# yassouali/pytorch-segmentation

Measured on NVIDIA H100. Metric: images/sec DeepLabV3+/ResNet101 513x513 train step (fwd+CE+bwd+SGD), higher is better.
Workload: dtype bf16

## Files before the change

### pytorch-segmentation_b200/csrc/seg_loss.cu

```cuda
#include "seg_common.cuh"

namespace seg {

__device__ __forceinline__ void block_accum2(double a, double b, double* out) {
  a = warp_sum_d(a);
  b = warp_sum_d(b);
  __shared__ double sa[32], sb[32];
  const int lane = threadIdx.x & 31, warp = threadIdx.x >> 5;
  if (lane == 0) {
    sa[warp] = a;
    sb[warp] = b;
  }
  __syncthreads();
  if (warp == 0) {
    const int nw = (blockDim.x + 31) >> 5;
    a = lane < nw ? sa[lane] : 0.0;
    b = lane < nw ? sb[lane] : 0.0;
    a = warp_sum_d(a);
    b = warp_sum_d(b);
    if (lane == 0) {
      atomicAdd(out, a);
      atomicAdd(out + 1, b);
    }
  }
// ... 93 lines not shown
                                                            int N, int C, int H, int W, double* accum) {
  const int64_t HW = (int64_t)H * W, total = (int64_t)N * HW;
  double inter = 0.0, psum = 0.0;
  for (int64_t i = blockIdx.x * (int64_t)blockDim.x + threadIdx.x; i < total; i += (int64_t)gridDim.x * blockDim.x) {
    const int64_t t = target[i];
    const int n = (int)(i / HW);
    const float* l = logits + (int64_t)n * C * HW + (i - (int64_t)n * HW);
    float mx = -INFINITY;
    for (int c = 0; c < C; ++c) mx = fmaxf(mx, l[(int64_t)c * HW]);
    float se = 0.f, et = 0.f;
    for (int c = 0; c < C; ++c) {
      const float e = expf(l[(int64_t)c * HW] - mx);
      se += e;
      if (c == t) et = e;
    }
    inter += (double)(et / se);
    psum += 1.0;
  }
  block_accum2(inter, psum, accum);
}

__global__ void __launch_bounds__(256) dice_nchw_bwd_kernel(const float* __restrict__ logits, const int64_t* __restrict__ target,
                                                            int N, int C, int H, int W, const double* __restrict__ accum,
                                                            float smooth, const float* __restrict__ gscale,
                                                            float* __restrict__ dl, float beta) {
  const int64_t HW = (int64_t)H * W, total = (int64_t)N * HW;
  const double D = accum[1] + accum[1] + (double)smooth;
  const float g = (gscale ? *gscale : 1.f) * (float)(-2.0 / D);
  for (int64_t i = blockIdx.x * (int64_t)blockDim.x + threadIdx.x; i < total; i += (int64_t)gridDim.x * blockDim.x) {
    const int64_t t = target[i];
    const int n = (int)(i / HW);
    const int64_t off = (int64_t)n * C * HW + (i - (int64_t)n * HW);
    const float* l = logits + off;
    float* d = dl + off;
    float mx = -INFINITY;
    for (int c = 0; c < C; ++c) mx = fmaxf(mx, l[(int64_t)c * HW]);
    float se = 0.f;
    for (int c = 0; c < C; ++c) se += expf(l[(int64_t)c * HW] - mx);
    const float inv = 1.f / se;
    const float pt = (t >= 0 && t < C) ? expf(l[t * HW] - mx) * inv : 0.f;
    for (int c = 0; c < C; ++c) {
      const float pc = expf(l[(int64_t)c * HW] - mx) * inv;
      const float v = g * pt * ((c == t ? 1.f : 0.f) - pc);
      d[(int64_t)c * HW] = (beta != 0.f) ? beta * d[(int64_t)c * HW] + v : v;
    }
  }
}

__global__ void dice_finalize_kernel(const double* accum, float smooth, float* loss) {
  if (threadIdx.x == 0 && blockIdx.x == 0)
    *loss = (float)(1.0 - (2.0 * accum[0] + smooth) / (accum[1] + accum[1] + smooth));
}

__global__ void loss_finalize_kernel(const double* accum, int mean, float* loss) {
  if (threadIdx.x == 0 && blockIdx.x == 0) *loss = (float)(!mean ? accum[0] : accum[1] > 0.0 ? accum[0] / accum[1] : 0.0);
}

struct Lerp2 {
  int i0, i1;
  float l1;
};
__device__ __forceinline__ Lerp2 src_idx(int dst, float scale, int in_size, int ac) {
  float s;
  if (ac) {
    s = scale * (float)dst;
  } else {
    s = scale * ((float)dst + 0.5f) - 0.5f;
    if (s < 0.f) s = 0.f;
  }
  Lerp2 r;
  r.i0 = (int)s;
  if (r.i0 > in_size - 1) r.i0 = in_size - 1;
  r.i1 = r.i0 + ((r.i0 < in_size - 1) ? 1 : 0);
  r.l1 = s - (float)r.i0;
  return r;
}
static inline float rscale(int in_size, int out_size, int ac) {
  if (ac) return out_size > 1 ? (float)(in_size - 1) / (float)(out_size - 1) : 0.f;
  return (float)in_size / (float)out_size;
}

constexpr int MAXC = 160;
constexpr int TILE = 32;

__device__ __forceinline__ double ce_grad_scale(double gmax, float sh, float sw, int Ho, int Wo) {
  const double ry = sh > 0.f ? 2.0 / sh : (double)Ho, rx = sw > 0.f ? 2.0 / sw : (double)Wo;
  int e;
  frexp(fabs(gmax) * (ry + 2.0) * (rx + 2.0), &e);
  return ldexp(1.0, 61 - e);
}
__device__ __forceinline__ float warp_weight_max(const float* w, int C) {
  float m = w ? 0.f : 1.f;
  if (w)
    for (int c = threadIdx.x & 31; c < C; c += 32) m = fmaxf(m, w[c]);
  for (int o = 16; o > 0; o >>= 1) m = fmaxf(m, __shfl_xor_sync(0xffffffffu, m, o));
  return m;
}
template <int K>
__device__ __forceinline__ double loss_grad_bound(float g, const LossArgs& la, int C) {
  if (K == LOSS_CE) return (double)g;
  return (double)g * (double)warp_weight_max(la.weight, C) * (K == LOSS_FOCAL ? 1.0 + (double)la.gamma : 1.0);
}
__device__ __forceinline__ unsigned long long to_fixed(float v, double scale) {
  return (unsigned long long)__double2ll_rn((double)v * scale);
}

template <bool BWD, int K, bool MET = false>
__global__ void __launch_bounds__(256) upsample_ce_kernel(const float* __restrict__ lo, const int64_t* __restrict__ target,
                                                          int N, int Hi, int Wi, int Ho, int Wo, int C, int ac, float sh,
                                                          float sw, int64_t ignore, LossArgs la, double* accum, int32_t* argmax,
                                                          const float* __restrict__ gscale,
                                                          unsigned long long* __restrict__ dlo_fixed, int patch, int tile,
                                                          unsigned long long* __restrict__ counters) {
  extern __shared__ unsigned long long sm64[];
  unsigned long long* dst = BWD ? sm64 : nullptr;
  float* src = reinterpret_cast<float*>(BWD ? sm64 + patch * patch * C : sm64);
  unsigned int* hist = MET ? reinterpret_cast<unsigned int*>(src + patch * patch * C) : nullptr;
  const int tiles_x = (Wo + tile - 1) / tile, tiles_y = (Ho + tile - 1) / tile;
  int t = blockIdx.x;
  const int tx = t % tiles_x;
  t /= tiles_x;
  const int ty = t % tiles_y;
  const int n = t / tiles_y;
  const int oy0 = ty * tile, ox0 = tx * tile;
  const int oy1 = min(oy0 + tile, Ho) - 1, ox1 = min(ox0 + tile, Wo) - 1;
  const int sy0 = src_idx(oy0, sh, Hi, ac).i0, sx0 = src_idx(ox0, sw, Wi, ac).i0;
  const int sy1 = src_idx(oy1, sh, Hi, ac).i1, sx1 = src_idx(ox1, sw, Wi, ac).i1;
  const int ph = sy1 - sy0 + 1, pw = sx1 - sx0 + 1;
  for (int i = threadIdx.x; i < ph * pw * C; i += blockDim.x) {
    const int c = i % C;
    const int pp = i / C;
    const int py = pp / pw, px = pp - py * pw;
    src[i] = lo[(((int64_t)n * Hi + sy0 + py) * Wi + sx0 + px) * C + c];
    if (BWD) dst[i] = 0ull;
  }
  if (MET)
    for (int i = threadIdx.x; i < 3 * C + 2; i += blockDim.x) hist[i] = 0u;
  __syncthreads();
  double loss = 0.0, cnt = 0.0;
  unsigned int n_correct = 0u, n_labeled = 0u;
  float g = 0.f;
  double scale = 0.0;
  if (BWD) {
    g = loss_grad_g<K>(gscale, accum, la.mean);
    scale = ce_grad_scale(loss_grad_bound<K>(g, la, C), sh, sw, Ho, Wo);
  }
  for (int e = threadIdx.x; e < tile * tile; e += blockDim.x) {
    const int oy = oy0 + e / tile, ox = ox0 + e % tile;
    if (oy >= Ho || ox >= Wo) continue;
    const int64_t tg = target[((int64_t)n * Ho + oy) * Wo + ox];
    const bool valid = tg != ignore;
    const bool labeled = MET && tg >= 0 && tg < C;
    if (K == LOSS_FOCAL && !BWD) cnt += 1.0;
    if (!valid && (BWD || (argmax == nullptr && !labeled))) continue;
    const Lerp2 ly = src_idx(oy, sh, Hi, ac), lx = src_idx(ox, sw, Wi, ac);
    const float h1 = ly.l1, h0 = 1.f - h1, w1 = lx.l1, w0 = 1.f - w1;
    const float* pa = src + ((ly.i0 - sy0) * pw + (lx.i0 - sx0)) * C;
    const float* pb = src + ((ly.i0 - sy0) * pw + (lx.i1 - sx0)) * C;
    const float* pc = src + ((ly.i1 - sy0) * pw + (lx.i0 - sx0)) * C;
    const float* pd = src + ((ly.i1 - sy0) * pw + (lx.i1 - sx0)) * C;
    float mx = -INFINITY;
    int am = 0;
    for (int c = 0; c < C; ++c) {
      const float v = h0 * (w0 * pa[c] + w1 * pb[c]) + h1 * (w0 * pc[c] + w1 * pd[c]);
      if (v > mx) {
        mx = v;
        am = c;
      }
    }
    float se = 0.f, lt = 0.f;
    for (int c = 0; c < C; ++c) {
      const float v = h0 * (w0 * pa[c] + w1 * pb[c]) + h1 * (w0 * pc[c] + w1 * pd[c]);
      se += expf(v - mx);
      if (c == tg) lt = v;
    }
    if (!BWD) {
      if (argmax) argmax[((int64_t)n * Ho + oy) * Wo + ox] = am;
      if (MET && labeled) {
        ++n_labeled;
        atomicAdd(&hist[2 + C + am], 1u);
        atomicAdd(&hist[2 + 2 * C + (int)tg], 1u);
        if (am == (int)tg) {
          ++n_correct;
          atomicAdd(&hist[2 + (int)tg], 1u);
        }
      }
      if (valid) {
        const float w = K == LOSS_CE ? 1.f : class_weight(la, tg, C);
        loss += (double)pixel_loss<K>(mx + logf(se) - lt, w, la.gamma);
        if (K == LOSS_CE) cnt += 1.0;
        if (K == LOSS_WCE) cnt += (double)w;
      }
    } else {
      const float inv = 1.f / se;
      const float gp = K == LOSS_CE ? g : g * pixel_grad_factor<K>(mx + logf(se) - lt, class_weight(la, tg, C), la.gamma);
      unsigned long long* da = dst + ((ly.i0 - sy0) * pw + (lx.i0 - sx0)) * C;
      unsigned long long* db = dst + ((ly.i0 - sy0) * pw + (lx.i1 - sx0)) * C;
      unsigned long long* dc = dst + ((ly.i1 - sy0) * pw + (lx.i0 - sx0)) * C;
      unsigned long long* dd = dst + ((ly.i1 - sy0) * pw + (lx.i1 - sx0)) * C;
      for (int c = 0; c < C; ++c) {
        const float v = h0 * (w0 * pa[c] + w1 * pb[c]) + h1 * (w0 * pc[c] + w1 * pd[c]);
        const float gr = (expf(v - mx) * inv - (c == tg ? 1.f : 0.f)) * gp;
        atomicAdd(da + c, to_fixed(h0 * w0 * gr, scale));
        atomicAdd(db + c, to_fixed(h0 * w1 * gr, scale));
        atomicAdd(dc + c, to_fixed(h1 * w0 * gr, scale));
        atomicAdd(dd + c, to_fixed(h1 * w1 * gr, scale));
      }
    }
  }
  if (!BWD) {
    block_accum2(loss, cnt, accum);
    if (MET) {
      n_correct = __reduce_add_sync(0xffffffffu, n_correct);
      n_labeled = __reduce_add_sync(0xffffffffu, n_labeled);
      if ((threadIdx.x & 31) == 0) {
        atomicAdd(&hist[0], n_correct);
        atomicAdd(&hist[1], n_labeled);
      }
      __syncthreads();
      for (int i = threadIdx.x; i < 3 * C + 2; i += blockDim.x) {
        const unsigned int v = hist[i];
        if (v != 0u) atomicAdd(counters + i, (unsigned long long)v);
      }
    }
  } else {
    __syncthreads();
    for (int i = threadIdx.x; i < ph * pw * C; i += blockDim.x) {
      const unsigned long long v = dst[i];
      if (v != 0ull) {
        const int c = i % C;
        const int pp = i / C;
        const int py = pp / pw, px = pp - py * pw;
        atomicAdd(dlo_fixed + (((int64_t)n * Hi + sy0 + py) * Wi + sx0 + px) * C + c, v);
      }
    }
  }
}

template <int K>
__global__ void ce_grad_from_fixed_kernel(const unsigned long long* __restrict__ acc, int64_t n, const float* gscale,
                                          const double* accum, LossArgs la, int C, float sh, float sw, int Ho, int Wo,
                                          float* __restrict__ dlo) {
  const double inv = 1.0 / ce_grad_scale(loss_grad_bound<K>(loss_grad_g<K>(gscale, accum, la.mean), la, C), sh, sw, Ho, Wo);
  for (int64_t i = blockIdx.x * (int64_t)blockDim.x + threadIdx.x; i < n; i += (int64_t)gridDim.x * blockDim.x)
    dlo[i] = (float)((double)(long long)acc[i] * inv);
}

__device__ __forceinline__ float logit_f(__nv_bfloat16 v) { return bf2f(v); }
__device__ __forceinline__ float logit_f(float v) { return v; }
template <bool BWD, int K, bool MET = false, typename T = __nv_bfloat16>
__global__ void __launch_bounds__(256) shuffle_ce_kernel(const T* __restrict__ lo, int ldlo,
                                                         const int64_t* __restrict__ target, int N, int h, int w, int C, int r,
                                                         int64_t ignore, LossArgs la, double* accum,
                                                         const float* __restrict__ gscale, __nv_bfloat16* __restrict__ dx,
                                                         int lddx, unsigned long long* __restrict__ counters) {
  extern __shared__ unsigned int hist[];
  if (MET) {
    for (int i = threadIdx.x; i < 3 * C + 2; i += blockDim.x) hist[i] = 0u;
    __syncthreads();
  }
  const int Ho = h * r, Wo = w * r, rr = r * r;
  const int64_t total = (int64_t)N * Ho * Wo;
  double loss = 0.0, cnt = 0.0;
  unsigned int n_correct = 0u, n_labeled = 0u;
  const float g = BWD ? loss_grad_g<K>(gscale, accum, la.mean) : 0.f;
  for (int64_t i = blockIdx.x * (int64_t)blockDim.x + threadIdx.x; i < total; i += (int64_t)gridDim.x * blockDim.x) {
    const int ox = (int)(i % Wo);
    const int64_t t = i / Wo;
    const int oy = (int)(t % Ho);
    const int n = (int)(t / Ho);
    const int64_t tg = target[i];
    const bool valid = tg != ignore;
    const bool labeled = MET && tg >= 0 && tg < C;
    if (K == LOSS_FOCAL && !BWD) cnt += 1.0;
    const int64_t px = ((int64_t)n * h + oy / r) * w + ox / r;
    const int sub = (oy % r) * r + ox % r;
    const T* z = lo + px * ldlo + sub;
    __nv_bfloat16* d = BWD ? dx + px * lddx + sub : nullptr;
    if (BWD) {
      if (sub == 0)
        for (int c = C * rr; c < lddx; ++c) d[c] = f2bf(0.f);
      if (!valid) {
        for (int c = 0; c < C; ++c) d[c * rr] = f2bf(0.f);
        continue;
      }
    } else if (!valid && !labeled) {
      continue;
    }
    float mx = -INFINITY;
    int am = 0;
    for (int c = 0; c < C; ++c) {
      const float v = logit_f(z[c * rr]);
      if (v > mx) {
        mx = v;
        am = c;
      }
    }
    float se = 0.f, lt = 0.f;
    for (int c = 0; c < C; ++c) {
      const float v = logit_f(z[c * rr]);
      se += expf(v - mx);
      if (c == tg) lt = v;
    }
    if (!BWD) {
      if (MET && labeled) {
        ++n_labeled;
        atomicAdd(&hist[2 + C + am], 1u);
        atomicAdd(&hist[2 + 2 * C + (int)tg], 1u);
        if (am == (int)tg) {
          ++n_correct;
          atomicAdd(&hist[2 + (int)tg], 1u);
        }
      }
      if (valid) {
        const float wt = K == LOSS_CE ? 1.f : class_weight(la, tg, C);
        loss += (double)pixel_loss<K>(mx + logf(se) - lt, wt, la.gamma);
        if (K == LOSS_CE) cnt += 1.0;
        if (K == LOSS_WCE) cnt += (double)wt;
      }
    } else {
      const float inv = 1.f / se;
      const float gp = K == LOSS_CE ? g : g * pixel_grad_factor<K>(mx + logf(se) - lt, class_weight(la, tg, C), la.gamma);
      for (int c = 0; c < C; ++c) {
        const float v = logit_f(z[c * rr]);
        d[c * rr] = f2bf((expf(v - mx) * inv - (c == tg ? 1.f : 0.f)) * gp);
      }
    }
  }
  if (!BWD) {
    block_accum2(loss, cnt, accum);
    if (MET) {
      n_correct = __reduce_add_sync(0xffffffffu, n_correct);
      n_labeled = __reduce_add_sync(0xffffffffu, n_labeled);
      if ((threadIdx.x & 31) == 0) {
        atomicAdd(&hist[0], n_correct);
        atomicAdd(&hist[1], n_labeled);
      }
      __syncthreads();
      for (int i = threadIdx.x; i < 3 * C + 2; i += blockDim.x) {
        const unsigned int v = hist[i];
        if (v != 0u) atomicAdd(counters + i, (unsigned long long)v);
      }
    }
  }
}

__global__ void cast_pad_kernel(const float* __restrict__ x, __nv_bfloat16* __restrict__ y, int64_t M, int C, int ld) {
  const int64_t total = M * ld;
  for (int64_t i = blockIdx.x * (int64_t)blockDim.x + threadIdx.x; i < total; i += (int64_t)gridDim.x * blockDim.x) {
    const int c = (int)(i % ld);
    const int64_t r = i / ld;
    y[i] = f2bf(c < C ? x[r * C + c] : 0.f);
  }
}

static int patch_for(int in_size, int out_size, int ac, int tile) {
  const float sc = rscale(in_size, out_size, ac);
  int p = (int)ceilf(sc * (tile - 1)) + 3;
  return p < in_size + 1 ? p : in_size + 1;
}

}

using namespace seg;
#define ST(s) reinterpret_cast<cudaStream_t>(s)

namespace seg {
template <int K>
static int ce_nchw_fwd(const float* logits, const int64_t* target, int N, int C, int H, int W, int64_t ignore_index,
                       LossArgs la, double* accum, cudaStream_t stream) {
  const int64_t total = (int64_t)N * H * W;
  int blocks = (int)std::min<int64_t>(ceil_div64(total, 256), (int64_t)num_sms() * 8);
  ce_nchw_fwd_kernel<K><<<blocks, 256, 0, stream>>>(logits, target, N, C, H, W, ignore_index, la, accum);
  return check_launch("ce_nchw_fwd");
}
template <int K>
static int ce_nchw_bwd(const float* logits, const int64_t* target, int N, int C, int H, int W, int64_t ignore_index,
                       LossArgs la, const double* accum, const float* gscale, float* dlogits, cudaStream_t stream) {
  const int64_t total = (int64_t)N * H * W;
  int blocks = (int)std::min<int64_t>(ceil_div64(total, 256), (int64_t)num_sms() * 8);
  ce_nchw_bwd_kernel<K><<<blocks, 256, 0, stream>>>(logits, target, N, C, H, W, ignore_index, la, accum, gscale, dlogits);
  return check_launch("ce_nchw_bwd");
}

template <int K>
static int upsample_ce_fwd(const float* logits_lo, const int64_t* target, int N, int Hi, int Wi, int Ho, int Wo, int C,
                           int align_corners, int64_t ignore_index, LossArgs la, double* accum, int32_t* argmax,
                           int64_t* counters, cudaStream_t stream) {
  SEG_REQUIRE(C <= MAXC, "upsample_ce: C=%d > %d", C, MAXC);
  const bool met = counters != nullptr;
  const auto kernel = met ? upsample_ce_kernel<false, K, true> : upsample_ce_kernel<false, K, false>;
  const int patch = std::max(patch_for(Hi, Ho, align_corners, TILE), patch_for(Wi, Wo, align_corners, TILE));
  const size_t smem = (size_t)patch * patch * C * sizeof(float) + (met ? (size_t)(3 * C + 2) * sizeof(unsigned int) : 0);
  SEG_REQUIRE(smem <= 200 * 1024, "upsample_ce: patch too large (%zu B)", smem);
  static size_t set_smem[2] = {0, 0};
  if (smem > set_smem[met]) {
    cudaFuncSetAttribute(kernel, cudaFuncAttributeMaxDynamicSharedMemorySize, (int)smem);
    set_smem[met] = smem;
  }
  const int blocks = N * ceil_div(Ho, TILE) * ceil_div(Wo, TILE);
  kernel<<<blocks, 256, smem, stream>>>(
      logits_lo, target, N, Hi, Wi, Ho, Wo, C, align_corners, rscale(Hi, Ho, align_corners), rscale(Wi, Wo, align_corners),
      ignore_index, la, accum, argmax, nullptr, nullptr, patch, TILE, reinterpret_cast<unsigned long long*>(counters));
  return check_launch(met ? "upsample_ce_fwd_metrics" : "upsample_ce_fwd");
}

template <int K>
static int upsample_ce_bwd(const float* logits_lo, const int64_t* target, int N, int Hi, int Wi, int Ho, int Wo, int C,
                           int align_corners, int64_t ignore_index, LossArgs la, const double* accum, const float* gscale,
                           float* dlo_f32, void* dlo_fixed, void* dx, int lddx, cudaStream_t stream) {
  SEG_REQUIRE(C <= MAXC, "upsample_ce: C=%d > %d", C, MAXC);
  auto bwd_patch = [&](int t) { return std::max(patch_for(Hi, Ho, align_corners, t), patch_for(Wi, Wo, align_corners, t)); };
  auto bwd_smem = [&](int t) { return (size_t)bwd_patch(t) * bwd_patch(t) * C * (sizeof(unsigned long long) + sizeof(float)); };
  const int tile = bwd_smem(TILE) <= 227 * 1024 ? TILE : TILE / 2;
  const int patch = bwd_patch(tile);
  const size_t smem = bwd_smem(tile);
  SEG_REQUIRE(smem <= 227 * 1024, "upsample_ce: patch too large (%zu B)", smem);
  static size_t set_smem = 0;
  if (smem > set_smem) {
    cudaFuncSetAttribute(upsample_ce_kernel<true, K>, cudaFuncAttributeMaxDynamicSharedMemorySize, (int)smem);
    set_smem = smem;
  }
  const int64_t M = (int64_t)N * Hi * Wi;
  unsigned long long* fixed = reinterpret_cast<unsigned long long*>(dlo_fixed);
  cudaMemsetAsync(fixed, 0, (size_t)M * C * sizeof(unsigned long long), stream);
  const int blocks = N * ceil_div(Ho, tile) * ceil_div(Wo, tile);
  const float sh = rscale(Hi, Ho, align_corners), sw = rscale(Wi, Wo, align_corners);
  upsample_ce_kernel<true, K><<<blocks, 256, smem, stream>>>(
      logits_lo, target, N, Hi, Wi, Ho, Wo, C, align_corners, sh, sw, ignore_index, la, const_cast<double*>(accum), nullptr,
      gscale, fixed, patch, tile, nullptr);
  if (check_launch("upsample_ce_bwd")) return 1;
  const int64_t n = M * C;
  ce_grad_from_fixed_kernel<K><<<(unsigned)std::min<int64_t>(ceil_div64(n, 256), (int64_t)num_sms() * 8), 256, 0, stream>>>(
      fixed, n, gscale, accum, la, C, sh, sw, Ho, Wo, dlo_f32);
  if (check_launch("ce_grad_from_fixed")) return 1;
  if (dx) {
    int blocks2 = (int)std::min<int64_t>(ceil_div64(M * lddx, 256), (int64_t)num_sms() * 8);
    cast_pad_kernel<<<blocks2, 256, 0, stream>>>(dlo_f32, reinterpret_cast<__nv_bfloat16*>(dx), M, C, lddx);
    return check_launch("cast_pad");
  }
  return 0;
}

static int shuffle_ce_check(int N, int h, int w, int C, int r, int ld) {
  SEG_REQUIRE(C <= MAXC, "shuffle_loss: C=%d > %d", C, MAXC);
  SEG_REQUIRE(N > 0 && h > 0 && w > 0 && r >= 1, "shuffle_loss: bad sizes");
  SEG_REQUIRE(ld >= C * r * r, "shuffle_loss: pitch %d < r*r*C = %d", ld, C * r * r);
  return 0;
}
static unsigned shuffle_ce_blocks(int N, int h, int w, int r) {
  return (unsigned)std::min<int64_t>(ceil_div64((int64_t)N * h * w * r * r, 256), (int64_t)num_sms() * 8);
}
template <int K, typename T = __nv_bfloat16>
static int shuffle_ce_fwd(const void* lo, int ldlo, const int64_t* target, int N, int h, int w, int C, int r, int64_t ignore_index,
                          LossArgs la, double* accum, int64_t* counters, cudaStream_t stream) {
  if (shuffle_ce_check(N, h, w, C, r, ldlo)) return 1;
  const bool met = counters != nullptr;
  const auto kernel = met ? shuffle_ce_kernel<false, K, true, T> : shuffle_ce_kernel<false, K, false, T>;
  kernel<<<shuffle_ce_blocks(N, h, w, r), 256, met ? (size_t)(3 * C + 2) * sizeof(unsigned int) : 0, stream>>>(
      reinterpret_cast<const T*>(lo), ldlo, target, N, h, w, C, r, ignore_index, la, accum, nullptr, nullptr, 0,
      reinterpret_cast<unsigned long long*>(counters));
  return check_launch(met ? "shuffle_ce_fwd_metrics" : "shuffle_ce_fwd");
}
template <int K, typename T = __nv_bfloat16>
static int shuffle_ce_bwd(const void* lo, int ldlo, const int64_t* target, int N, int h, int w, int C, int r, int64_t ignore_index,
                          LossArgs la, const double* accum, const float* gscale, void* dx, int lddx, cudaStream_t stream) {
  if (shuffle_ce_check(N, h, w, C, r, ldlo) || shuffle_ce_check(N, h, w, C, r, lddx)) return 1;
  shuffle_ce_kernel<true, K, false, T><<<shuffle_ce_blocks(N, h, w, r), 256, 0, stream>>>(
      reinterpret_cast<const T*>(lo), ldlo, target, N, h, w, C, r, ignore_index, la, const_cast<double*>(accum),
      gscale, reinterpret_cast<__nv_bfloat16*>(dx), lddx, nullptr);
  return check_launch("shuffle_ce_bwd");
}
template <int K>
static int nhwc_ce_fwd(const float* logits, int ld, const int64_t* target, int N, int H, int W, int C, int64_t ignore_index,
                       LossArgs la, double* accum, int64_t* counters, cudaStream_t stream) {
  return shuffle_ce_fwd<K, float>(logits, ld, target, N, H, W, C, 1, ignore_index, la, accum, counters, stream);
}
template <int K>
static int nhwc_ce_bwd(const float* logits, int ld, const int64_t* target, int N, int H, int W, int C, int64_t ignore_index,
                       LossArgs la, const double* accum, const float* gscale, void* dx, int lddx, cudaStream_t stream) {
  return shuffle_ce_bwd<K, float>(logits, ld, target, N, H, W, C, 1, ignore_index, la, accum, gscale, dx, lddx, stream);
}

static int loss_args(const float* weight, int kind, float gamma, int mean, int C, LossArgs* la) {
  SEG_REQUIRE(C > 0, "loss: C=%d", C);
  SEG_REQUIRE(kind == LOSS_CE || kind == LOSS_WCE || kind == LOSS_FOCAL, "loss: unknown kind %d", kind);
  SEG_REQUIRE(kind != LOSS_CE || (weight == nullptr && mean), "loss: SEG_LOSS_CE takes no class weight and is a mean");
  SEG_REQUIRE(kind != LOSS_FOCAL || (gamma >= 0.f && isfinite(gamma)), "loss: focal gamma must be finite and >= 0 (got %g)",
              (double)gamma);
  *la = LossArgs{weight, gamma, mean ? 1 : 0};
  return 0;
}
#define SEG_LOSS_DISPATCH(kind, fn, ...)                   \
  ((kind) == LOSS_CE    ? fn<LOSS_CE>(__VA_ARGS__)         \
   : (kind) == LOSS_WCE ? fn<LOSS_WCE>(__VA_ARGS__)        \
                        : fn<LOSS_FOCAL>(__VA_ARGS__))
}

extern "C" {

int seg_loss_nchw_fwd(const float* logits, const int64_t* target, int N, int C, int H, int W, int64_t ignore_index,
                      const float* weight, int kind, float gamma, double* accum, void* stream) {
  LossArgs la;
  if (loss_args(weight, kind, gamma, 1, C, &la)) return 1;
  return SEG_LOSS_DISPATCH(kind, ce_nchw_fwd, logits, target, N, C, H, W, ignore_index, la, accum, ST(stream));
}
int seg_loss_nchw_bwd(const float* logits, const int64_t* target, int N, int C, int H, int W, int64_t ignore_index,
                      const float* weight, int kind, float gamma, int mean, const double* accum, const float* gscale,
                      float* dlogits, void* stream) {
  LossArgs la;
  if (loss_args(weight, kind, gamma, mean, C, &la)) return 1;
  return SEG_LOSS_DISPATCH(kind, ce_nchw_bwd, logits, target, N, C, H, W, ignore_index, la, accum, gscale, dlogits, ST(stream));
}
int seg_dice_nchw_fwd(const float* logits, const int64_t* target, int N, int C, int H, int W, float smooth, double* accum,
                      float* loss, void* stream) {
  const int64_t total = (int64_t)N * H * W;
  int blocks = (int)std::min<int64_t>(ceil_div64(total, 256), (int64_t)num_sms() * 8);
  dice_nchw_fwd_kernel<<<blocks, 256, 0, ST(stream)>>>(logits, target, N, C, H, W, accum);
  if (check_launch("dice_nchw_fwd")) return 1;
  dice_finalize_kernel<<<1, 32, 0, ST(stream)>>>(accum, smooth, loss);
  return check_launch("dice_finalize");
}
int seg_dice_nchw_bwd(const float* logits, const int64_t* target, int N, int C, int H, int W, const double* accum,
                      float smooth, const float* gscale, float* dlogits, float beta, void* stream) {
  const int64_t total = (int64_t)N * H * W;
  int blocks = (int)std::min<int64_t>(ceil_div64(total, 256), (int64_t)num_sms() * 8);
  dice_nchw_bwd_kernel<<<blocks, 256, 0, ST(stream)>>>(logits, target, N, C, H, W, accum, smooth, gscale, dlogits, beta);
  return check_launch("dice_nchw_bwd");
}
int seg_loss_finalize(const double* accum, int mean, float* loss, void* stream) {
  loss_finalize_kernel<<<1, 32, 0, ST(stream)>>>(accum, mean, loss);
  return check_launch("loss_finalize");
}

int seg_upsample_loss_fwd(const float* logits_lo, const int64_t* target, int N, int Hi, int Wi, int Ho, int Wo, int C,
                          int align_corners, int64_t ignore_index, const float* weight, int kind, float gamma, double* accum,
                          int32_t* argmax, int64_t* counters, void* stream) {
  LossArgs la;
  if (loss_args(weight, kind, gamma, 1, C, &la)) return 1;
  return SEG_LOSS_DISPATCH(kind, upsample_ce_fwd, logits_lo, target, N, Hi, Wi, Ho, Wo, C, align_corners, ignore_index, la, accum,
                           argmax, counters, ST(stream));
}
int seg_upsample_loss_bwd(const float* logits_lo, const int64_t* target, int N, int Hi, int Wi, int Ho, int Wo, int C,
                          int align_corners, int64_t ignore_index, const float* weight, int kind, float gamma, int mean,
                          const double* accum, const float* gscale, float* dlo_f32, void* dlo_fixed, void* dx, int lddx,
                          void* stream) {
  LossArgs la;
  if (loss_args(weight, kind, gamma, mean, C, &la)) return 1;
  return SEG_LOSS_DISPATCH(kind, upsample_ce_bwd, logits_lo, target, N, Hi, Wi, Ho, Wo, C, align_corners, ignore_index, la, accum,
                           gscale, dlo_f32, dlo_fixed, dx, lddx, ST(stream));
}

int seg_shuffle_loss_fwd(const void* logits_lo, int ldlo, const int64_t* target, int N, int h, int w, int C, int r,
                         int64_t ignore_index, const float* weight, int kind, float gamma, double* accum, int64_t* counters,
                         void* stream) {
  LossArgs la;
  if (loss_args(weight, kind, gamma, 1, C, &la)) return 1;
  return SEG_LOSS_DISPATCH(kind, shuffle_ce_fwd, logits_lo, ldlo, target, N, h, w, C, r, ignore_index, la, accum, counters,
                           ST(stream));
}
int seg_shuffle_loss_bwd(const void* logits_lo, int ldlo, const int64_t* target, int N, int h, int w, int C, int r,
                         int64_t ignore_index, const float* weight, int kind, float gamma, int mean, const double* accum,
                         const float* gscale, void* dx, int lddx, void* stream) {
  LossArgs la;
  if (loss_args(weight, kind, gamma, mean, C, &la)) return 1;
  return SEG_LOSS_DISPATCH(kind, shuffle_ce_bwd, logits_lo, ldlo, target, N, h, w, C, r, ignore_index, la, accum, gscale, dx, lddx,
                           ST(stream));
}

int seg_nhwc_loss_fwd(const float* logits, int ld, const int64_t* target, int N, int H, int W, int C, int64_t ignore_index,
                      const float* weight, int kind, float gamma, double* accum, int64_t* counters, void* stream) {
  LossArgs la;
  if (loss_args(weight, kind, gamma, 1, C, &la)) return 1;
  return SEG_LOSS_DISPATCH(kind, nhwc_ce_fwd, logits, ld, target, N, H, W, C, ignore_index, la, accum, counters, ST(stream));
}
int seg_nhwc_loss_bwd(const float* logits, int ld, const int64_t* target, int N, int H, int W, int C, int64_t ignore_index,
                      const float* weight, int kind, float gamma, int mean, const double* accum, const float* gscale, void* dx,
                      int lddx, void* stream) {
  LossArgs la;
  if (loss_args(weight, kind, gamma, mean, C, &la)) return 1;
  return SEG_LOSS_DISPATCH(kind, nhwc_ce_bwd, logits, ld, target, N, H, W, C, ignore_index, la, accum, gscale, dx, lddx,
                           ST(stream));
}

}

namespace seg {
__global__ void __launch_bounds__(256)
    eval_metrics_kernel(const float* __restrict__ logits, const int64_t* __restrict__ target, int N, int C, int64_t HW, int K,
                        unsigned long long* __restrict__ out) {
  extern __shared__ unsigned int hist[];
  for (int i = threadIdx.x; i < 3 * K + 2; i += blockDim.x) hist[i] = 0u;
  __syncthreads();
  const int64_t total = (int64_t)N * HW;
  for (int64_t i = blockIdx.x * (int64_t)blockDim.x + threadIdx.x; i < total; i += (int64_t)gridDim.x * blockDim.x) {
    const int64_t t = target[i];
    if (t < 0 || t >= K) continue;
    const int n = (int)(i / HW);
    const float* l = logits + (int64_t)n * C * HW + (i - (int64_t)n * HW);
    float best = l[0];
    int arg = 0;
    for (int c = 1; c < C; ++c) {
      const float v = l[(int64_t)c * HW];
      if (v > best) {
        best = v;
        arg = c;
      }
    }
    atomicAdd(&hist[3 * K + 1], 1u);
    if (arg < K) atomicAdd(&hist[K + arg], 1u);
    atomicAdd(&hist[2 * K + (int)t], 1u);
    if (arg == (int)t) {
      atomicAdd(&hist[3 * K], 1u);
      atomicAdd(&hist[(int)t], 1u);
    }
  }
  __syncthreads();
  for (int i = threadIdx.x; i < 3 * K + 2; i += blockDim.x) {
    const unsigned int v = hist[i];
    if (v == 0u) continue;
    const int dst = (i == 3 * K) ? 0 : (i == 3 * K + 1) ? 1 : 2 + i;
    atomicAdd(out + dst, (unsigned long long)v);
  }
}
}

extern "C" int seg_eval_metrics_nchw(const float* logits, const int64_t* target, int N, int C, int H, int W, int num_class,
                                     int64_t* out, void* stream) {
  using namespace seg;
  SEG_REQUIRE(N > 0 && C > 0 && num_class > 0 && num_class <= 4096, "eval_metrics: bad sizes (C=%d num_class=%d)", C, num_class);
  cudaStream_t st = reinterpret_cast<cudaStream_t>(stream);
  cudaMemsetAsync(out, 0, (size_t)(2 + 3 * num_class) * sizeof(int64_t), st);
  const int64_t HW = (int64_t)H * W, total = (int64_t)N * HW;
// ... 8 lines not shown
```

### pytorch-segmentation_b200/seg_b200/ops.py

```python
import ctypes

import torch

from . import lib
from .lib import DT_BF16, DT_F32, IMPL_AUTO, IMPL_SIMT, IMPL_TC, ConvDesc, call, make_conv_desc, ptr

_IMPL_OVERRIDE = None
PROFILE = None


def _meta(d):
    if lib.TRACE is None:
        return None
    return (d.N, d.H, d.W, d.C, d.K, d.R, d.stride, d.dil, 2.0 * d.N * d.P * d.Q * d.K * d.C * d.R * d.S)


def _meta_rows(M, C, passes, flag=0):
    if lib.TRACE is None:
        return None
    return (int(M), int(C), int(flag), 0, 0, 0, 0, 0, 2.0 * M * C * passes)


def _prof(kind, d):
    if PROFILE is None:
# ... 533 lines not shown


def loss_nchw_bwd(logits, target, ignore_index, accum, weight=None, gamma=None, mean=True, gscale=None):
    N, C, H, W = logits.shape
    dl = torch.empty_like(logits)
    call("seg_loss_nchw_bwd", ptr(logits), ptr(target), N, C, H, W, int(ignore_index), ptr(weight), _loss_kind(weight, gamma, mean),
         float(gamma or 0.0), int(mean), ptr(accum), ptr(gscale), ptr(dl))
    return dl


def dice_nchw_fwd(logits, target, smooth=1.0):
    N, C, H, W = logits.shape
    assert logits.is_contiguous() and logits.dtype == torch.float32 and target.dtype == torch.int64 and target.is_contiguous()
    accum = torch.zeros(2, dtype=torch.float64, device=logits.device)
    loss = torch.empty((), dtype=torch.float32, device=logits.device)
    call("seg_dice_nchw_fwd", ptr(logits), ptr(target), N, C, H, W, float(smooth), ptr(accum), ptr(loss))
    return loss, accum


def dice_nchw_bwd(logits, target, accum, smooth=1.0, gscale=None, out=None, beta=0.0):
    N, C, H, W = logits.shape
    if out is None:
        out = torch.empty_like(logits)
        beta = 0.0
    call("seg_dice_nchw_bwd", ptr(logits), ptr(target), N, C, H, W, ptr(accum), float(smooth), ptr(gscale), ptr(out), float(beta))
    return out


def lovasz_softmax_nchw(logits, target, ignore_index):
    N, C, H, W = logits.shape
    assert logits.is_contiguous() and logits.dtype == torch.float32 and target.dtype == torch.int64 and target.is_contiguous()
    dev = logits.device
    counts = torch.empty(C + 1, dtype=torch.int32, device=dev)
    call("seg_lovasz_count", ptr(target), N * H * W, C, int(ignore_index), ptr(counts))
    ch = counts.cpu()
    P, n_present = int(ch[C]), int((ch[:C] > 0).sum())
    nkeys = max(P * n_present, 1)
    keys0 = torch.empty(nkeys, dtype=torch.int64, device=dev)
    keys1 = torch.empty(nkeys, dtype=torch.int64, device=dev)
    ws = torch.empty(int(lib.load().seg_lovasz_workspace_bytes(P, n_present, C)), dtype=torch.uint8, device=dev)
    loss = torch.empty((), dtype=torch.float32, device=dev)
    dl = torch.empty_like(logits)
    call("seg_lovasz_softmax_nchw", ptr(logits), ptr(target), N, C, H, W, int(ignore_index), ptr(counts), P, n_present,
         ptr(keys0), ptr(keys1), ptr(ws), ptr(loss), ptr(dl))
    return loss, dl


def eval_metrics_nchw(logits, target, num_class):
    N, C, H, W = logits.shape
    assert logits.is_contiguous() and logits.dtype == torch.float32 and target.dtype == torch.int64 and target.is_contiguous()
    out = torch.empty(2 + 3 * num_class, dtype=torch.int64, device=logits.device)
    call("seg_eval_metrics_nchw", ptr(logits), ptr(target), N, C, H, W, int(num_class), ptr(out))
    return out


def _check_counters(counters, C):
    assert counters.dtype == torch.int64 and counters.is_contiguous() and counters.numel() == 2 + 3 * C


def upsample_loss_fwd(logits_lo, target, align_corners, ignore_index, weight=None, gamma=None, mean=True, want_argmax=False,
                      reduce_fn=None, counters=None):
    N, Hi, Wi, C = logits_lo.shape
    _, Ho, Wo = target.shape
    assert logits_lo.is_contiguous() and logits_lo.dtype == torch.float32 and target.is_contiguous()
    assert weight is None or (weight.dtype == torch.float32 and weight.numel() == C and weight.is_contiguous())
    if counters is not None:
        _check_counters(counters, C)
    accum = torch.zeros(2, dtype=torch.float64, device=logits_lo.device)
    am = torch.empty((N, Ho, Wo), dtype=torch.int32, device=logits_lo.device) if want_argmax else None
    call("seg_upsample_loss_fwd", ptr(logits_lo), ptr(target), N, Hi, Wi, Ho, Wo, C, int(align_corners), int(ignore_index),
         ptr(weight), _loss_kind(weight, gamma, mean), float(gamma or 0.0), ptr(accum), ptr(am), ptr(counters))
    if reduce_fn is not None:
        reduce_fn(accum)
    loss = torch.empty((), dtype=torch.float32, device=logits_lo.device)
    call("seg_loss_finalize", ptr(accum), int(mean), ptr(loss))
    return loss, accum, am


def upsample_loss_bwd(logits_lo, target, align_corners, ignore_index, accum, ldx, weight=None, gamma=None, mean=True,
                      gscale=None):
    N, Hi, Wi, C = logits_lo.shape
    _, Ho, Wo = target.shape
    dlo = torch.empty((N, Hi, Wi, C), dtype=torch.float32, device=logits_lo.device)
    fixed = torch.empty((N, Hi, Wi, C), dtype=torch.int64, device=logits_lo.device)
    dx = torch.empty((N, Hi, Wi, ldx), dtype=torch.bfloat16, device=logits_lo.device)
    call("seg_upsample_loss_bwd", ptr(logits_lo), ptr(target), N, Hi, Wi, Ho, Wo, C, int(align_corners), int(ignore_index),
         ptr(weight), _loss_kind(weight, gamma, mean), float(gamma or 0.0), int(mean), ptr(accum), ptr(gscale), ptr(dlo),
         ptr(fixed), ptr(dx), ldx)
    return dx, dlo


def _shuffle_loss_shapes(lo, r, target):
    N, h, w, Cr = lo.shape
    C = Cr // (r * r)
    assert C * r * r == Cr and lo.dtype == torch.bfloat16 and target.dtype == torch.int64 and target.is_contiguous()
    if tuple(target.shape) != (N, h * r, w * r):
        raise ValueError(f"target size {tuple(target.shape[1:])} differs from the model output size {(h * r, w * r)}")
    return N, h, w, C


def shuffle_loss_fwd(logits_lo, r, target, ignore_index, weight=None, gamma=None, mean=True, reduce_fn=None, counters=None):
    N, h, w, C = _shuffle_loss_shapes(logits_lo, r, target)
    assert weight is None or (weight.dtype == torch.float32 and weight.numel() == C and weight.is_contiguous())
    if counters is not None:
        _check_counters(counters, C)
    accum = torch.zeros(2, dtype=torch.float64, device=logits_lo.device)
    call("seg_shuffle_loss_fwd", ptr(logits_lo), ld(logits_lo), ptr(target), N, h, w, C, r, int(ignore_index), ptr(weight),
         _loss_kind(weight, gamma, mean), float(gamma or 0.0), ptr(accum), ptr(counters))
    if reduce_fn is not None:
        reduce_fn(accum)
    loss = torch.empty((), dtype=torch.float32, device=logits_lo.device)
    call("seg_loss_finalize", ptr(accum), int(mean), ptr(loss))
    return loss, accum


def shuffle_loss_bwd(logits_lo, r, target, ignore_index, accum, ldx, weight=None, gamma=None, mean=True, gscale=None):
    N, h, w, C = _shuffle_loss_shapes(logits_lo, r, target)
    dx = torch.empty((N, h, w, ldx), dtype=torch.bfloat16, device=logits_lo.device)
    call("seg_shuffle_loss_bwd", ptr(logits_lo), ld(logits_lo), ptr(target), N, h, w, C, r, int(ignore_index), ptr(weight),
         _loss_kind(weight, gamma, mean), float(gamma or 0.0), int(mean), ptr(accum), ptr(gscale), ptr(dx), ldx)
    return dx


def _nhwc_loss_shapes(logits, target):
    N, H, W, C = logits.shape
    assert logits.dtype == torch.float32 and target.dtype == torch.int64 and target.is_contiguous()
    if tuple(target.shape) != (N, H, W):
        raise ValueError(f"target size {tuple(target.shape[1:])} differs from the model output size {(H, W)}")
    return N, H, W, C


def nhwc_loss_fwd(logits, target, ignore_index, weight=None, gamma=None, mean=True, reduce_fn=None, counters=None):
    N, H, W, C = _nhwc_loss_shapes(logits, target)
    assert weight is None or (weight.dtype == torch.float32 and weight.numel() == C and weight.is_contiguous())
    if counters is not None:
        _check_counters(counters, C)
    accum = torch.zeros(2, dtype=torch.float64, device=logits.device)
    call("seg_nhwc_loss_fwd", ptr(logits), ld(logits), ptr(target), N, H, W, C, int(ignore_index), ptr(weight),
         _loss_kind(weight, gamma, mean), float(gamma or 0.0), ptr(accum), ptr(counters))
    if reduce_fn is not None:
        reduce_fn(accum)
    loss = torch.empty((), dtype=torch.float32, device=logits.device)
    call("seg_loss_finalize", ptr(accum), int(mean), ptr(loss))
    return loss, accum


def nhwc_loss_bwd(logits, target, ignore_index, accum, ldx, weight=None, gamma=None, mean=True, gscale=None):
    N, H, W, C = _nhwc_loss_shapes(logits, target)
    dx = torch.empty((N, H, W, ldx), dtype=torch.bfloat16, device=logits.device)
    call("seg_nhwc_loss_bwd", ptr(logits), ld(logits), ptr(target), N, H, W, C, int(ignore_index), ptr(weight),
         _loss_kind(weight, gamma, mean), float(gamma or 0.0), int(mean), ptr(accum), ptr(gscale), ptr(dx), ldx)
    return dx


def nhwc_to_nchw_f32(x):
    N, H, W, C = x.shape
    y = torch.empty((N, C, H, W), dtype=torch.float32, device=x.device)
    call("seg_nhwc_to_nchw_f32", ptr(x), ld(x), DT_BF16 if x.dtype == torch.bfloat16 else DT_F32, ptr(y), N, H, W, C)
    return y


def relu_fwd(x):
    y = torch.empty(x.shape, dtype=torch.bfloat16, device=x.device)
    call("seg_relu_fwd", ptr(x), ld(x), ptr(y), ld(y), rows(x), x.shape[-1])
    return y


def relu_bwd(dy, y, dx, beta):
    call("seg_relu_bwd", ptr(dy), ld(dy), ptr(y), ld(y), ptr(dx), ld(dx), rows(y), y.shape[-1], float(beta))
    return dx

# ... 120 lines not shown
```

Baseline: 381.5.

## Rewrite upsample CE backward as gather over low-res tiles, fusing conversion

Replaces the scatter-style backward of the bilinear upsample + cross-entropy loss, which did shared and global 64-bit fixed-point atomics into a full-size int64 buffer, with a gather kernel. Each block owns an 8x8 low-resolution tile, computes per-pixel gradients for the output pixels that reach it in shared-memory chunks, and sums contributions deterministically. The fixed-to-float conversion and bf16 cast/pad happen in the same kernel, which removes the memset, the int64 buffer and two extra launches. In exchange, output pixels near tile borders have their softmax recomputed by neighbouring blocks, and register caps are forced with __maxnreg__.

```diff
diff --git a/pytorch-segmentation_b200/csrc/seg_loss.cu b/pytorch-segmentation_b200/csrc/seg_loss.cu
--- a/pytorch-segmentation_b200/csrc/seg_loss.cu
+++ b/pytorch-segmentation_b200/csrc/seg_loss.cu
@@ -199,6 +199,7 @@
 
 constexpr int MAXC = 160;
 constexpr int TILE = 32;
+constexpr int GT = 8;
 
 __device__ __forceinline__ double ce_grad_scale(double gmax, float sh, float sw, int Ho, int Wo) {
   const double ry = sh > 0.f ? 2.0 / sh : (double)Ho, rx = sw > 0.f ? 2.0 / sw : (double)Wo;
@@ -222,16 +223,13 @@
   return (unsigned long long)__double2ll_rn((double)v * scale);
 }
 
-template <bool BWD, int K, bool MET = false>
+template <int K, bool MET = false>
 __global__ void __launch_bounds__(256) upsample_ce_kernel(const float* __restrict__ lo, const int64_t* __restrict__ target,
                                                           int N, int Hi, int Wi, int Ho, int Wo, int C, int ac, float sh,
                                                           float sw, int64_t ignore, LossArgs la, double* accum, int32_t* argmax,
-                                                          const float* __restrict__ gscale,
-                                                          unsigned long long* __restrict__ dlo_fixed, int patch, int tile,
-                                                          unsigned long long* __restrict__ counters) {
+                                                          int patch, int tile, unsigned long long* __restrict__ counters) {
   extern __shared__ unsigned long long sm64[];
-  unsigned long long* dst = BWD ? sm64 : nullptr;
-  float* src = reinterpret_cast<float*>(BWD ? sm64 + patch * patch * C : sm64);
+  float* src = reinterpret_cast<float*>(sm64);
   unsigned int* hist = MET ? reinterpret_cast<unsigned int*>(src + patch * patch * C) : nullptr;
   const int tiles_x = (Wo + tile - 1) / tile, tiles_y = (Ho + tile - 1) / tile;
   int t = blockIdx.x;
@@ -249,27 +247,20 @@
     const int pp = i / C;
     const int py = pp / pw, px = pp - py * pw;
     src[i] = lo[(((int64_t)n * Hi + sy0 + py) * Wi + sx0 + px) * C + c];
-    if (BWD) dst[i] = 0ull;
   }
   if (MET)
     for (int i = threadIdx.x; i < 3 * C + 2; i += blockDim.x) hist[i] = 0u;
   __syncthreads();
   double loss = 0.0, cnt = 0.0;
   unsigned int n_correct = 0u, n_labeled = 0u;
-  float g = 0.f;
-  double scale = 0.0;
-  if (BWD) {
-    g = loss_grad_g<K>(gscale, accum, la.mean);
-    scale = ce_grad_scale(loss_grad_bound<K>(g, la, C), sh, sw, Ho, Wo);
-  }
   for (int e = threadIdx.x; e < tile * tile; e += blockDim.x) {
     const int oy = oy0 + e / tile, ox = ox0 + e % tile;
     if (oy >= Ho || ox >= Wo) continue;
     const int64_t tg = target[((int64_t)n * Ho + oy) * Wo + ox];
     const bool valid = tg != ignore;
     const bool labeled = MET && tg >= 0 && tg < C;
-    if (K == LOSS_FOCAL && !BWD) cnt += 1.0;
-    if (!valid && (BWD || (argmax == nullptr && !labeled))) continue;
+    if (K == LOSS_FOCAL) cnt += 1.0;
+    if (!valid && argmax == nullptr && !labeled) continue;
     const Lerp2 ly = src_idx(oy, sh, Hi, ac), lx = src_idx(ox, sw, Wi, ac);
     const float h1 = ly.l1, h0 = 1.f - h1, w1 = lx.l1, w0 = 1.f - w1;
     const float* pa = src + ((ly.i0 - sy0) * pw + (lx.i0 - sx0)) * C;
@@ -291,76 +282,170 @@
       se += expf(v - mx);
       if (c == tg) lt = v;
     }
-    if (!BWD) {
-      if (argmax) argmax[((int64_t)n * Ho + oy) * Wo + ox] = am;
-      if (MET && labeled) {
-        ++n_labeled;
-        atomicAdd(&hist[2 + C + am], 1u);
-        atomicAdd(&hist[2 + 2 * C + (int)tg], 1u);
-        if (am == (int)tg) {
-          ++n_correct;
-          atomicAdd(&hist[2 + (int)tg], 1u);
-        }
-      }
-      if (valid) {
-        const float w = K == LOSS_CE ? 1.f : class_weight(la, tg, C);
-        loss += (double)pixel_loss<K>(mx + logf(se) - lt, w, la.gamma);
-        if (K == LOSS_CE) cnt += 1.0;
-        if (K == LOSS_WCE) cnt += (double)w;
-      }
+    if (argmax) argmax[((int64_t)n * Ho + oy) * Wo + ox] = am;
+    if (MET && labeled) {
+      ++n_labeled;
+      atomicAdd(&hist[2 + C + am], 1u);
+      atomicAdd(&hist[2 + 2 * C + (int)tg], 1u);
+      if (am == (int)tg) {
+        ++n_correct;
+        atomicAdd(&hist[2 + (int)tg], 1u);
+      }
+    }
+    if (valid) {
+      const float w = K == LOSS_CE ? 1.f : class_weight(la, tg, C);
+      loss += (double)pixel_loss<K>(mx + logf(se) - lt, w, la.gamma);
+      if (K == LOSS_CE) cnt += 1.0;
+      if (K == LOSS_WCE) cnt += (double)w;
+    }
+  }
+  block_accum2(loss, cnt, accum);
+  if (MET) {
+    n_correct = __reduce_add_sync(0xffffffffu, n_correct);
+    n_labeled = __reduce_add_sync(0xffffffffu, n_labeled);
+    if ((threadIdx.x & 31) == 0) {
+      atomicAdd(&hist[0], n_correct);
+      atomicAdd(&hist[1], n_labeled);
+    }
+    __syncthreads();
+    for (int i = threadIdx.x; i < 3 * C + 2; i += blockDim.x) {
+      const unsigned int v = hist[i];
+      if (v != 0u) atomicAdd(counters + i, (unsigned long long)v);
+    }
+  }
+}
+
+__device__ __forceinline__ int first_dst(int v, bool hi, float scale, int in_size, int out_size, int ac) {
+  int a = 0, b = out_size;
+  while (a < b) {
+    const int m = (a + b) >> 1;
+    const Lerp2 l = src_idx(m, scale, in_size, ac);
+    if ((hi ? l.i1 : l.i0) >= v) b = m;
+    else a = m + 1;
+  }
+  return a;
+}
+
+template <int K>
+__global__ void __maxnreg__(K == LOSS_FOCAL ? 72 : 64) upsample_ce_grad_kernel(const float* __restrict__ lo, const int64_t* __restrict__ target,
+                                                               int Hi, int Wi, int Ho, int Wo, int C, int ac, float sh, float sw,
+                                                               int64_t ignore, LossArgs la, const double* __restrict__ accum,
+                                                               const float* __restrict__ gscale, float* __restrict__ dlo,
+                                                               __nv_bfloat16* __restrict__ dx, int lddx, int chunk) {
+  extern __shared__ unsigned long long sm64[];
+  const int CP = C | 1;
+  unsigned long long* acc = sm64;
+  float4* hw = reinterpret_cast<float4*>(sm64 + GT * GT * C);
+  float* src = reinterpret_cast<float*>(hw + chunk);
+  float* gr = src + (GT + 2) * (GT + 2) * CP;
+  __shared__ int yr[2][GT][2], xr[2][GT][2];
+  const int tiles_x = (Wi + GT - 1) / GT, tiles_y = (Hi + GT - 1) / GT;
+  int t = blockIdx.x;
+  const int tx = t % tiles_x;
+  t /= tiles_x;
+  const int ty = t % tiles_y;
+  const int n = t / tiles_y;
+  const int ty0 = ty * GT, tx0 = tx * GT;
+  const int th = min(GT, Hi - ty0), tw = min(GT, Wi - tx0), tpc = th * tw * C;
+  if (threadIdx.x < 4 * GT) {
+    const int p = threadIdx.x % GT, hi = (threadIdx.x / GT) & 1;
+    int* r = threadIdx.x < 2 * GT ? yr[hi][p] : xr[hi][p];
+    if (threadIdx.x < 2 * GT) {
+      r[0] = first_dst(ty0 + p, hi, sh, Hi, Ho, ac);
+      r[1] = first_dst(ty0 + p + 1, hi, sh, Hi, Ho, ac);
     } else {
+      r[0] = first_dst(tx0 + p, hi, sw, Wi, Wo, ac);
+      r[1] = first_dst(tx0 + p + 1, hi, sw, Wi, Wo, ac);
+    }
+  }
+  const int ry0 = first_dst(ty0, true, sh, Hi, Ho, ac), ry1 = first_dst(ty0 + th, false, sh, Hi, Ho, ac);
+  const int rx0 = first_dst(tx0, true, sw, Wi, Wo, ac), rx1 = first_dst(tx0 + tw, false, sw, Wi, Wo, ac);
+  const bool reached = ry1 > ry0 && rx1 > rx0;
+  int sy0 = 0, sx0 = 0, pw = 0;
+  if (reached) {
+    sy0 = src_idx(ry0, sh, Hi, ac).i0;
+    sx0 = src_idx(rx0, sw, Wi, ac).i0;
+    const int ph = src_idx(ry1 - 1, sh, Hi, ac).i1 - sy0 + 1;
+    pw = src_idx(rx1 - 1, sw, Wi, ac).i1 - sx0 + 1;
+    for (int i = threadIdx.x; i < ph * pw * C; i += blockDim.x) {
+      const int c = i % C, pp = i / C;
+      const int py = pp / pw, px = pp - py * pw;
+      src[pp * CP + c] = lo[(((int64_t)n * Hi + sy0 + py) * Wi + sx0 + px) * C + c];
+    }
+  }
+  for (int i = threadIdx.x; i < tpc; i += blockDim.x) acc[i] = 0ull;
+  const float g = loss_grad_g<K>(gscale, accum, la.mean);
+  const double scale = ce_grad_scale(loss_grad_bound<K>(g, la, C), sh, sw, Ho, Wo);
+  __syncthreads();
+  const int cwmax = reached ? min(rx1 - rx0, chunk) : 1;
+  for (int cx0 = rx0; reached && cx0 < rx1; cx0 += cwmax)
+  for (int cy0 = ry0, cw = min(cwmax, rx1 - cx0); cy0 < ry1; cy0 += chunk / cw) {
+    const int rows = min(chunk / cw, ry1 - cy0), nk = rows * cw;
+    for (int k = threadIdx.x; k < nk; k += blockDim.x) {
+      const int oy = cy0 + k / cw, ox = cx0 + k % cw;
+      const int64_t tg = target[((int64_t)n * Ho + oy) * Wo + ox];
+      const Lerp2 ly = src_idx(oy, sh, Hi, ac), lx = src_idx(ox, sw, Wi, ac);
+      const float h1 = ly.l1, h0 = 1.f - h1, w1 = lx.l1, w0 = 1.f - w1;
+      hw[k] = make_float4(__fmul_rn(h0, w0), __fmul_rn(h0, w1), __fmul_rn(h1, w0), __fmul_rn(h1, w1));
+      float* d = gr + k * CP;
+      if (tg == ignore) {
+        for (int c = 0; c < C; ++c) d[c] = 0.f;
+        continue;
+      }
+      const float* pa = src + ((ly.i0 - sy0) * pw + (lx.i0 - sx0)) * CP;
+      const float* pb = src + ((ly.i0 - sy0) * pw + (lx.i1 - sx0)) * CP;
+      const float* pc = src + ((ly.i1 - sy0) * pw + (lx.i0 - sx0)) * CP;
+      const float* pd = src + ((ly.i1 - sy0) * pw + (lx.i1 - sx0)) * CP;
+      float mx = -INFINITY;
+      for (int c = 0; c < C; ++c) {
+        const float v = __fmaf_rn(h0, __fmaf_rn(w0, pa[c], __fmul_rn(w1, pb[c])), __fmul_rn(h1, __fmaf_rn(w0, pc[c], __fmul_rn(w1, pd[c]))));
+        d[c] = v;
+        if (v > mx) mx = v;
+      }
+      float se = 0.f, lt = 0.f;
+      for (int c = 0; c < C; ++c) {
+        const float v = d[c];
+        se += expf(v - mx);
+        if (c == tg) lt = v;
+      }
       const float inv = 1.f / se;
       const float gp = K == LOSS_CE ? g : g * pixel_grad_factor<K>(mx + logf(se) - lt, class_weight(la, tg, C), la.gamma);
-      unsigned long long* da = dst + ((ly.i0 - sy0) * pw + (lx.i0 - sx0)) * C;
-      unsigned long long* db = dst + ((ly.i0 - sy0) * pw + (lx.i1 - sx0)) * C;
-      unsigned long long* dc = dst + ((ly.i1 - sy0) * pw + (lx.i0 - sx0)) * C;
-      unsigned long long* dd = dst + ((ly.i1 - sy0) * pw + (lx.i1 - sx0)) * C;
-      for (int c = 0; c < C; ++c) {
-        const float v = h0 * (w0 * pa[c] + w1 * pb[c]) + h1 * (w0 * pc[c] + w1 * pd[c]);
-        const float gr = (expf(v - mx) * inv - (c == tg ? 1.f : 0.f)) * gp;
-        atomicAdd(da + c, to_fixed(h0 * w0 * gr, scale));
-        atomicAdd(db + c, to_fixed(h0 * w1 * gr, scale));
-        atomicAdd(dc + c, to_fixed(h1 * w0 * gr, scale));
-        atomicAdd(dd + c, to_fixed(h1 * w1 * gr, scale));
-      }
-    }
-  }
-  if (!BWD) {
-    block_accum2(loss, cnt, accum);
-    if (MET) {
-      n_correct = __reduce_add_sync(0xffffffffu, n_correct);
-      n_labeled = __reduce_add_sync(0xffffffffu, n_labeled);
-      if ((threadIdx.x & 31) == 0) {
-        atomicAdd(&hist[0], n_correct);
-        atomicAdd(&hist[1], n_labeled);
-      }
-      __syncthreads();
-      for (int i = threadIdx.x; i < 3 * C + 2; i += blockDim.x) {
-        const unsigned int v = hist[i];
-        if (v != 0u) atomicAdd(counters + i, (unsigned long long)v);
-      }
-    }
-  } else {
+      for (int c = 0; c < C; ++c) d[c] = __fmul_rn(__fmaf_rn(expf(d[c] - mx), inv, c == tg ? -1.f : -0.f), gp);
+    }
     __syncthreads();
-    for (int i = threadIdx.x; i < ph * pw * C; i += blockDim.x) {
-      const unsigned long long v = dst[i];
-      if (v != 0ull) {
-        const int c = i % C;
-        const int pp = i / C;
-        const int py = pp / pw, px = pp - py * pw;
-        atomicAdd(dlo_fixed + (((int64_t)n * Hi + sy0 + py) * Wi + sx0 + px) * C + c, v);
-      }
-    }
-  }
-}
-
-template <int K>
-__global__ void ce_grad_from_fixed_kernel(const unsigned long long* __restrict__ acc, int64_t n, const float* gscale,
-                                          const double* accum, LossArgs la, int C, float sh, float sw, int Ho, int Wo,
-                                          float* __restrict__ dlo) {
-  const double inv = 1.0 / ce_grad_scale(loss_grad_bound<K>(loss_grad_g<K>(gscale, accum, la.mean), la, C), sh, sw, Ho, Wo);
-  for (int64_t i = blockIdx.x * (int64_t)blockDim.x + threadIdx.x; i < n; i += (int64_t)gridDim.x * blockDim.x)
-    dlo[i] = (float)((double)(long long)acc[i] * inv);
+    for (int e = threadIdx.x; e < tpc; e += blockDim.x) {
+      const int c = e % C, p = e / C;
+      const int py = p / tw, px = p - py * tw;
+      const int xa0 = max(xr[0][px][0], cx0) - cx0, xb0 = min(xr[0][px][1], cx0 + cw) - cx0;
+      const int xa1 = max(xr[1][px][0], cx0) - cx0, xb1 = min(xr[1][px][1], cx0 + cw) - cx0;
+      const float* g0 = gr + c;
+      unsigned long long s = 0ull;
+      for (int ys = 0; ys < 2; ++ys) {
+        const int ya = max(yr[ys][py][0], cy0), yb = min(yr[ys][py][1], cy0 + rows);
+        const float* q = reinterpret_cast<const float*>(hw) + 2 * ys;
+        for (int oy = ya; oy < yb; ++oy) {
+          const int base = (oy - cy0) * cw;
+          for (int k = base + xa0; k < base + xb0; ++k) s += to_fixed(__fmul_rn(q[4 * k], g0[k * CP]), scale);
+          for (int k = base + xa1; k < base + xb1; ++k) s += to_fixed(__fmul_rn(q[4 * k + 1], g0[k * CP]), scale);
+        }
+      }
+      acc[e] += s;
+    }
+    __syncthreads();
+  }
+  const double inv = 1.0 / scale;
+  for (int e = threadIdx.x; e < tpc; e += blockDim.x) {
+    const int c = e % C, p = e / C;
+    const int py = p / tw, px = p - py * tw;
+    dlo[(((int64_t)n * Hi + ty0 + py) * Wi + tx0 + px) * C + c] = (float)((double)(long long)acc[e] * inv);
+  }
+  if (dx)
+    for (int e = threadIdx.x; e < th * tw * lddx; e += blockDim.x) {
+      const int c = e % lddx, p = e / lddx;
+      const int py = p / tw, px = p - py * tw;
+      dx[(((int64_t)n * Hi + ty0 + py) * Wi + tx0 + px) * lddx + c] =
+          f2bf(c < C ? (float)((double)(long long)acc[p * C + c] * inv) : 0.f);
+    }
 }
 
 __device__ __forceinline__ float logit_f(__nv_bfloat16 v) { return bf2f(v); }
@@ -462,15 +547,6 @@
   }
 }
 
-__global__ void cast_pad_kernel(const float* __restrict__ x, __nv_bfloat16* __restrict__ y, int64_t M, int C, int ld) {
-  const int64_t total = M * ld;
-  for (int64_t i = blockIdx.x * (int64_t)blockDim.x + threadIdx.x; i < total; i += (int64_t)gridDim.x * blockDim.x) {
-    const int c = (int)(i % ld);
-    const int64_t r = i / ld;
-    y[i] = f2bf(c < C ? x[r * C + c] : 0.f);
-  }
-}
-
 static int patch_for(int in_size, int out_size, int ac, int tile) {
   const float sc = rscale(in_size, out_size, ac);
   int p = (int)ceilf(sc * (tile - 1)) + 3;
@@ -506,7 +582,7 @@
                            int64_t* counters, cudaStream_t stream) {
   SEG_REQUIRE(C <= MAXC, "upsample_ce: C=%d > %d", C, MAXC);
   const bool met = counters != nullptr;
-  const auto kernel = met ? upsample_ce_kernel<false, K, true> : upsample_ce_kernel<false, K, false>;
+  const auto kernel = met ? upsample_ce_kernel<K, true> : upsample_ce_kernel<K, false>;
   const int patch = std::max(patch_for(Hi, Ho, align_corners, TILE), patch_for(Wi, Wo, align_corners, TILE));
   const size_t smem = (size_t)patch * patch * C * sizeof(float) + (met ? (size_t)(3 * C + 2) * sizeof(unsigned int) : 0);
   SEG_REQUIRE(smem <= 200 * 1024, "upsample_ce: patch too large (%zu B)", smem);
@@ -518,45 +594,30 @@
   const int blocks = N * ceil_div(Ho, TILE) * ceil_div(Wo, TILE);
   kernel<<<blocks, 256, smem, stream>>>(
       logits_lo, target, N, Hi, Wi, Ho, Wo, C, align_corners, rscale(Hi, Ho, align_corners), rscale(Wi, Wo, align_corners),
-      ignore_index, la, accum, argmax, nullptr, nullptr, patch, TILE, reinterpret_cast<unsigned long long*>(counters));
+      ignore_index, la, accum, argmax, patch, TILE, reinterpret_cast<unsigned long long*>(counters));
   return check_launch(met ? "upsample_ce_fwd_metrics" : "upsample_ce_fwd");
 }
 
 template <int K>
 static int upsample_ce_bwd(const float* logits_lo, const int64_t* target, int N, int Hi, int Wi, int Ho, int Wo, int C,
                            int align_corners, int64_t ignore_index, LossArgs la, const double* accum, const float* gscale,
-                           float* dlo_f32, void* dlo_fixed, void* dx, int lddx, cudaStream_t stream) {
+                           float* dlo, void* dx, int lddx, cudaStream_t stream) {
   SEG_REQUIRE(C <= MAXC, "upsample_ce: C=%d > %d", C, MAXC);
-  auto bwd_patch = [&](int t) { return std::max(patch_for(Hi, Ho, align_corners, t), patch_for(Wi, Wo, align_corners, t)); };
-  auto bwd_smem = [&](int t) { return (size_t)bwd_patch(t) * bwd_patch(t) * C * (sizeof(unsigned long long) + sizeof(float)); };
-  const int tile = bwd_smem(TILE) <= 227 * 1024 ? TILE : TILE / 2;
-  const int patch = bwd_patch(tile);
-  const size_t smem = bwd_smem(tile);
-  SEG_REQUIRE(smem <= 227 * 1024, "upsample_ce: patch too large (%zu B)", smem);
+  const int CP = C | 1;
+  const size_t fixed = (size_t)GT * GT * C * sizeof(unsigned long long) + (size_t)(GT + 2) * (GT + 2) * CP * sizeof(float);
+  const size_t per_px = sizeof(float4) + (size_t)CP * sizeof(float), budget = 226 * 1024;
+  const int chunk = (int)std::min<size_t>(256, (budget - fixed) / per_px / 32 * 32);
+  const size_t smem = fixed + chunk * per_px;
   static size_t set_smem = 0;
   if (smem > set_smem) {
-    cudaFuncSetAttribute(upsample_ce_kernel<true, K>, cudaFuncAttributeMaxDynamicSharedMemorySize, (int)smem);
+    cudaFuncSetAttribute(upsample_ce_grad_kernel<K>, cudaFuncAttributeMaxDynamicSharedMemorySize, (int)smem);
     set_smem = smem;
   }
-  const int64_t M = (int64_t)N * Hi * Wi;
-  unsigned long long* fixed = reinterpret_cast<unsigned long long*>(dlo_fixed);
-  cudaMemsetAsync(fixed, 0, (size_t)M * C * sizeof(unsigned long long), stream);
-  const int blocks = N * ceil_div(Ho, tile) * ceil_div(Wo, tile);
-  const float sh = rscale(Hi, Ho, align_corners), sw = rscale(Wi, Wo, align_corners);
-  upsample_ce_kernel<true, K><<<blocks, 256, smem, stream>>>(
-      logits_lo, target, N, Hi, Wi, Ho, Wo, C, align_corners, sh, sw, ignore_index, la, const_cast<double*>(accum), nullptr,
-      gscale, fixed, patch, tile, nullptr);
-  if (check_launch("upsample_ce_bwd")) return 1;
-  const int64_t n = M * C;
-  ce_grad_from_fixed_kernel<K><<<(unsigned)std::min<int64_t>(ceil_div64(n, 256), (int64_t)num_sms() * 8), 256, 0, stream>>>(
-      fixed, n, gscale, accum, la, C, sh, sw, Ho, Wo, dlo_f32);
-  if (check_launch("ce_grad_from_fixed")) return 1;
-  if (dx) {
-    int blocks2 = (int)std::min<int64_t>(ceil_div64(M * lddx, 256), (int64_t)num_sms() * 8);
-    cast_pad_kernel<<<blocks2, 256, 0, stream>>>(dlo_f32, reinterpret_cast<__nv_bfloat16*>(dx), M, C, lddx);
-    return check_launch("cast_pad");
-  }
-  return 0;
+  const int blocks = N * ceil_div(Hi, GT) * ceil_div(Wi, GT);
+  upsample_ce_grad_kernel<K><<<blocks, 256, smem, stream>>>(
+      logits_lo, target, Hi, Wi, Ho, Wo, C, align_corners, rscale(Hi, Ho, align_corners), rscale(Wi, Wo, align_corners),
+      ignore_index, la, accum, gscale, dlo, reinterpret_cast<__nv_bfloat16*>(dx), lddx, chunk);
+  return check_launch("upsample_ce_bwd");
 }
 
 static int shuffle_ce_check(int N, int h, int w, int C, int r, int ld) {
@@ -664,8 +725,9 @@
                           void* stream) {
   LossArgs la;
   if (loss_args(weight, kind, gamma, mean, C, &la)) return 1;
+  (void)dlo_fixed;
   return SEG_LOSS_DISPATCH(kind, upsample_ce_bwd, logits_lo, target, N, Hi, Wi, Ho, Wo, C, align_corners, ignore_index, la, accum,
-                           gscale, dlo_f32, dlo_fixed, dx, lddx, ST(stream));
+                           gscale, dlo_f32, dx, lddx, ST(stream));
 }
 
 int seg_shuffle_loss_fwd(const void* logits_lo, int ldlo, const int64_t* target, int N, int h, int w, int C, int r,
diff --git a/pytorch-segmentation_b200/seg_b200/ops.py b/pytorch-segmentation_b200/seg_b200/ops.py
--- a/pytorch-segmentation_b200/seg_b200/ops.py
+++ b/pytorch-segmentation_b200/seg_b200/ops.py
@@ -639,11 +639,10 @@
     N, Hi, Wi, C = logits_lo.shape
     _, Ho, Wo = target.shape
     dlo = torch.empty((N, Hi, Wi, C), dtype=torch.float32, device=logits_lo.device)
-    fixed = torch.empty((N, Hi, Wi, C), dtype=torch.int64, device=logits_lo.device)
     dx = torch.empty((N, Hi, Wi, ldx), dtype=torch.bfloat16, device=logits_lo.device)
     call("seg_upsample_loss_bwd", ptr(logits_lo), ptr(target), N, Hi, Wi, Ho, Wo, C, int(align_corners), int(ignore_index),
          ptr(weight), _loss_kind(weight, gamma, mean), float(gamma or 0.0), int(mean), ptr(accum), ptr(gscale), ptr(dlo),
-         ptr(fixed), ptr(dx), ldx)
+         None, ptr(dx), ldx)
     return dx, dlo
 
 
```

Measured after the change: 386.9, median of 6. 1.4% higher.
